# rll/rllab

Hardware: NVIDIA H100
Metric: env-steps/sec (full iteration: rollout + process_samples + VPG update) (higher is better)
Workload: dtype f32

## Files before the change

rllab_b200/csrc/tile_gram.cuh:

```cuda
#pragma once
#include "update_common.cuh"

namespace b200rl {

constexpr int TILE_AMAX = 6;
struct TileDist {
  float ls_new[TILE_AMAX], inv_std[TILE_AMAX], ls_old[TILE_AMAX], inv_std_old[TILE_AMAX], Mmu[TILE_AMAX],
      var_new[TILE_AMAX], var_new2[TILE_AMAX], var_old[TILE_AMAX];
  float sum_ls_new, sum_ls_old, half_log2pi_A;
};

template <class N, int MODE>
__device__ __forceinline__ void tile_dist_init(TileDist& D, const float* log_std_params, const UpdArgs& a) {
  constexpr int A = N::A;
  static_assert(A <= TILE_AMAX, "act_dim beyond the TileDist arrays");
  D.sum_ls_new = 0.f;
  D.sum_ls_old = 0.f;
#pragma unroll
  for (int k = 0; k < A; ++k) {
    D.ls_new[k] = clamp_log_std(log_std_params[k], a.log_min_std);
    const float sd = expf(D.ls_new[k]);
    D.inv_std[k] = 1.0f / sd;
    D.var_new[k] = sd * sd;
    D.var_new2[k] = 2.0f * sd * sd + 1e-8f;
    D.Mmu[k] = 2.0f / D.var_new2[k];
    D.ls_old[k] = (MODE == MODE_FVP) ? D.ls_new[k] : a.old_log_std[k];
    const float so = expf(D.ls_old[k]);
    D.inv_std_old[k] = 1.0f / so;
    D.var_old[k] = so * so;
    D.sum_ls_new += D.ls_new[k];
    D.sum_ls_old += D.ls_old[k];
  }
  D.half_log2pi_A = 0.5f * (float)A * 1.8378770664093453f;
}

template <class N, int RX, int RH1, int RH2, int RD1, int RD2, int RDM, int LD, bool PACKED = false, int TILE = 128>
struct TileGram {
  static constexpr int O = N::O, H = 32, A = N::A;
  static_assert(TILE == 128 || TILE == 64, "128- or 64-sample stages");
  static constexpr int WC = TILE == 128 ? 4 : 2;
  static constexpr int CS = 32 / WC;
  static constexpr int OQ = (O + 3) / 4;
  static_assert(N::H1 == 32 && N::H2 == 32 && A <= 6, "32-wide layers, act_dim <= 6");
  static constexpr int NS = A <= 3 ? 1 : 2;
  static constexpr int JDB = A <= 3 ? 3 : A;
  double accW1[4][WC];
  double accB[OQ + 1];
  double accA, accA1;
  double accT;
  float pA[NS][2], pT, pB[OQ + 1];

  __device__ __forceinline__ static void w1_tile_of(int tid, int& ti, int& tj, int& kh) {
    if constexpr (TILE == 128) {
      ti = (tid & 63) >> 3;
      tj = tid & 7;
      kh = tid >> 6;
    } else {
      ti = tid & 7;
      tj = tid >> 3;
      kh = 0;
    }
  }

  __device__ __forceinline__ void zero_partials() {
#pragma unroll
    for (int s = 0; s < NS; ++s) pA[s][0] = pA[s][1] = 0.f;
    pT = 0.f;
#pragma unroll
    for (int i = 0; i <= OQ; ++i) pB[i] = 0.f;
  }

  __device__ __forceinline__ void init() {
#pragma unroll
    for (int r = 0; r < 4; ++r)
#pragma unroll
      for (int c = 0; c < WC; ++c) accW1[r][c] = 0.0;
#pragma unroll
    for (int k = 0; k <= OQ; ++k) accB[k] = 0.0;
    accA = 0.0;
    accA1 = 0.0;
    accT = 0.0;
    zero_partials();
  }

  __device__ __forceinline__ void accumulate_a(const float* stage, int tid) {
    part_a(stage, tid);
    fold_a(tid);
  }
  __device__ __forceinline__ void accumulate_b(const float* stage, int tid) {
    part_b<LD>(stage, stage + RX * LD, tid);
    fold_b();
  }

  __device__ __forceinline__ void part_a(const float* stage, int tid) {
    int ti, tj, kh;
    w1_tile_of(tid, ti, tj, kh);
    const float* U = stage + (RH1 + ti) * LD + kh * 64;
    const float* V = stage + (RD2 + tj) * LD + kh * 64;
    if constexpr (PACKED) {
      float2 acc[4][WC];
#pragma unroll
      for (int r = 0; r < 4; ++r)
#pragma unroll
        for (int c = 0; c < WC; ++c) acc[r][c] = make_float2(0.f, 0.f);
#pragma unroll 2
      for (int k = 0; k < 64; k += 4) {
        float4 u[4], v[WC];
#pragma unroll
        for (int r = 0; r < 4; ++r) u[r] = *reinterpret_cast<const float4*>(U + r * 8 * LD + k);
#pragma unroll
        for (int c = 0; c < WC; ++c) v[c] = *reinterpret_cast<const float4*>(V + c * CS * LD + k);
#pragma unroll
        for (int r = 0; r < 4; ++r)
#pragma unroll
          for (int c = 0; c < WC; ++c) gram_fma4(u[r], v[c], acc[r][c]);
      }
#pragma unroll
      for (int r = 0; r < 4; ++r)
#pragma unroll
        for (int c = 0; c < WC; ++c) accW1[r][c] += (double)(acc[r][c].x + acc[r][c].y);
    } else {
      float acc[4][WC];
#pragma unroll
      for (int r = 0; r < 4; ++r)
#pragma unroll
        for (int c = 0; c < WC; ++c) acc[r][c] = 0.f;
#pragma unroll 4
      for (int k = 0; k < 64; k += 4) {
        float4 u[4], v[WC];
#pragma unroll
        for (int r = 0; r < 4; ++r) u[r] = *reinterpret_cast<const float4*>(U + r * 8 * LD + k);
#pragma unroll
        for (int c = 0; c < WC; ++c) v[c] = *reinterpret_cast<const float4*>(V + c * CS * LD + k);
#pragma unroll
        for (int r = 0; r < 4; ++r)
#pragma unroll
          for (int c = 0; c < WC; ++c) {
            acc[r][c] = fmaf(u[r].x, v[c].x, acc[r][c]);
            acc[r][c] = fmaf(u[r].y, v[c].y, acc[r][c]);
            acc[r][c] = fmaf(u[r].z, v[c].z, acc[r][c]);
            acc[r][c] = fmaf(u[r].w, v[c].w, acc[r][c]);
          }
      }
#pragma unroll
      for (int r = 0; r < 4; ++r)
#pragma unroll
        for (int c = 0; c < WC; ++c) accW1[r][c] += (double)acc[r][c];
    }
    const int lane = tid & 31, wq = tid >> 5;
#pragma unroll
    for (int s = 0; s < NS; ++s) {
    const int j = wq + 4 * s;
    if (j < A) {
      const float* Hh = stage + (RH2 + lane) * LD;
      const float* M = stage + (RDM + j) * LD;
      float s0 = pA[s][0], s1 = pA[s][1];
#pragma unroll 4
      for (int k = 0; k < TILE; k += 4) {
        const float4 hv = *reinterpret_cast<const float4*>(Hh + k);
        const float4 m = *reinterpret_cast<const float4*>(M + k);
        s0 = fmaf(hv.x, m.x, s0); s1 = fmaf(hv.y, m.y, s1);
        s0 = fmaf(hv.z, m.z, s0); s1 = fmaf(hv.w, m.w, s1);
      }
      pA[s][0] = s0;
      pA[s][1] = s1;
    } else if (j == JDB) {
      const float* Dr = stage + (RD2 + lane) * LD;
      float s0 = pA[s][0];
#pragma unroll 4
      for (int k = 0; k < TILE; k += 4) {
        const float4 d = *reinterpret_cast<const float4*>(Dr + k);
        s0 += (d.x + d.y) + (d.z + d.w);
      }
      pA[s][0] = s0;
    }
    }
    if (tid < 2 * A) {
      const float* Dr = stage + (RDM + tid) * LD;
      float s0 = pT;
#pragma unroll 4
      for (int k = 0; k < TILE; k += 4) {
        const float4 d = *reinterpret_cast<const float4*>(Dr + k);
        s0 += (d.x + d.y) + (d.z + d.w);
      }
      pT = s0;
    }
  }

  __device__ __forceinline__ void fold_a(int tid) {
    const int wq = tid >> 5;
#pragma unroll
    for (int s = 0; s < NS; ++s) {
      const int j = wq + 4 * s;
      double& acc = s == 0 ? accA : accA1;
      if (j < A) acc += (double)(pA[s][0] + pA[s][1]);
      else if (j == JDB) acc += (double)pA[s][0];
      pA[s][0] = pA[s][1] = 0.f;
    }
    if (tid < 2 * A) accT += (double)pT;
    pT = 0.f;
  }

  template <int XLD>
  __device__ __forceinline__ void part_b(const float* stage, const float* X, int tid) {
    const int lane = tid & 31, wq = tid >> 5;
    const float* Dr = stage + (RD1 + lane) * LD;
    float sa[OQ + 1];
#pragma unroll
    for (int i = 0; i <= OQ; ++i) sa[i] = pB[i];
#pragma unroll 4
    for (int k = 0; k < TILE; k += 4) {
      const float4 d = *reinterpret_cast<const float4*>(Dr + k);
#pragma unroll
      for (int i = 0; i < OQ; ++i) {
        const int o = wq + 4 * i;
        if (o < O) {
          const float4 xv = *reinterpret_cast<const float4*>(X + o * XLD + k);
          sa[i] = fmaf(xv.x, d.x, sa[i]); sa[i] = fmaf(xv.y, d.y, sa[i]);
          sa[i] = fmaf(xv.z, d.z, sa[i]); sa[i] = fmaf(xv.w, d.w, sa[i]);
        }
      }
      if (wq == 3) sa[OQ] += (d.x + d.y) + (d.z + d.w);
    }
#pragma unroll
    for (int i = 0; i <= OQ; ++i) pB[i] = sa[i];
  }

  __device__ __forceinline__ void fold_b() {
#pragma unroll
    for (int i = 0; i <= OQ; ++i) {
      accB[i] += (double)pB[i];
      pB[i] = 0.f;
    }
  }

  __device__ __forceinline__ void write(double* out, double* scr, int tid) {
    write(out, scr, tid, [] { __syncthreads(); });
  }
  template <class Sync>
  __device__ __forceinline__ void write(double* out, double* scr, int tid, Sync sync) {
    int ti, tj, kh;
    w1_tile_of(tid, ti, tj, kh);
    if constexpr (TILE == 128) {
      const int w1_tile = tid & 63;
#pragma unroll
      for (int r = 0; r < 4; ++r)
#pragma unroll
        for (int c = 0; c < 4; ++c) scr[(kh * 64 + w1_tile) * 16 + r * 4 + c] = accW1[r][c];
      sync();
      if (tid < 64) {
#pragma unroll
        for (int r = 0; r < 4; ++r)
#pragma unroll
          for (int c = 0; c < 4; ++c)
            out[N::oW1 + (ti + 8 * r) * H + (tj + 8 * c)] = scr[w1_tile * 16 + r * 4 + c] + scr[(64 + w1_tile) * 16 + r * 4 + c];
      }
    } else {
#pragma unroll
      for (int r = 0; r < 4; ++r)
#pragma unroll
        for (int c = 0; c < WC; ++c) out[N::oW1 + (ti + 8 * r) * H + (tj + CS * c)] = accW1[r][c];
    }
    const int lane = tid & 31, wq = tid >> 5;
#pragma unroll
    for (int i = 0; i < OQ; ++i) {
      const int o = wq + 4 * i;
      if (o < O) out[N::oW0 + o * H + lane] = accB[i];
    }
    if constexpr (A <= 3) {
      if (wq == 3) {
        out[N::ob0 + lane] = accB[OQ];
        out[N::ob1 + lane] = accA;
      } else if (wq < A) {
        out[N::oWo + lane * A + wq] = accA;
      }
    } else {
      if (wq == 3) out[N::ob0 + lane] = accB[OQ];
#pragma unroll
      for (int s = 0; s < NS; ++s) {
        const int j = wq + 4 * s;
        const double acc = s == 0 ? accA : accA1;
        if (j == JDB) out[N::ob1 + lane] = acc;
        else if (j < A) out[N::oWo + lane * A + j] = acc;
      }
    }
    if (tid < 2 * A) out[N::obo + tid] = accT;
  }
};

}
```

rllab_b200/csrc/update_umma32.cu:

```cuda
#include "tile_gram.cuh"
#include "umma_common.cuh"

namespace b200rl {

constexpr int V_THREADS = 128, V_TILE = 128, V_LD = V_TILE + 4;
#ifndef B200RL_V_PACKED_GRAM
#define B200RL_V_PACKED_GRAM 1
#endif
#ifndef B200RL_V_NWG_GRAD
#define B200RL_V_NWG_GRAD 4
#endif

template <class N, int MODE>
struct Umma32 {
  static constexpr int O = N::O, H = 32, A = N::A;
  static_assert(N::H1 == 32 && N::H2 == 32 && O <= 24, "tensor-core 32-wide kernel: (32,32) nets, obs_dim <= 24");
  static constexpr int KX = ((O + 7) / 8) * 8;
  static constexpr int IMG = 32 * 32 * 4, IMGX = 32 * KX * 4;
  static constexpr int o_bXT = 0, o_bW1T = o_bXT + 2 * IMGX, o_bW1 = o_bW1T + 2 * IMG,
                       o_bV1T = o_bW1 + (MODE == MODE_LOSS ? 0 : 2 * IMG),
                       o_img_end = o_bV1T + (MODE == MODE_FVP ? 2 * IMG : 0);
  static constexpr int n_small = ((64 + 2 * H * A + A + 3) / 4) * 4;
  static constexpr int o_small = o_img_end, o_stage = o_small + n_small * 4;
  static constexpr bool BLK = is_grad_mode(MODE) && A == 1;
  static constexpr int NB = BLK ? 1 : 2;
  static constexpr int NWG = BLK ? B200RL_V_NWG_GRAD : MODE == MODE_LOSS ? 3 : 2;
  static constexpr bool SEP_D1 = BLK && NWG <= 4;
  static constexpr int LD = NB * 64 + 4;
  static constexpr int rH1 = 0, rH2 = rH1 + H, rD2 = rH2 + H, rDM = rD2 + H, rDL = rDM + A,
                       rD1 = SEP_D1 ? rDL + A : rH2, R = (MODE == MODE_LOSS) ? 0 : SEP_D1 ? rD1 + H : rDL + A;
  static constexpr int RR = O + (MODE == MODE_FVP ? 0 : 2 * A + 1), qX = 0, qAct = O, qOm = O + A, qAdv = O + 2 * A;
  static constexpr int w_red = ((R * LD * 4 + 15) / 16) * 16, w_ring = w_red + 3 * 32 * 8,
                       w_bytes = w_ring + 2 * RR * V_LD * 4;
  static constexpr int o_dist = ((o_stage + 15) / 16) * 16;
  static constexpr int o_wg = ((o_dist + (int)sizeof(TileDist) + 15) / 16) * 16;
  static_assert(MODE == MODE_LOSS || BLK || 2 * 64 * 16 * 8 <= R * LD * 4, "stage region must hold the K-half combine scratch");
  static constexpr size_t bytes = (size_t)o_wg + (size_t)NWG * w_bytes;
  static_assert(bytes <= 232448, "does not fit the 227 KB of shared memory");
};

__device__ __forceinline__ void v_wg_sync(int wg) { asm volatile("bar.sync %0, 128;" ::"r"(wg + 1) : "memory"); }

template <int K, bool IS_MAX>
__device__ __forceinline__ void v_wg_reduce_store(const double (&v)[K], double* scratch, double* out, int tid, int wg) {
  const int lane = tid & 31, warp = tid >> 5;
#pragma unroll
  for (int k = 0; k < K; ++k) {
    double s = IS_MAX ? warp_max(v[k]) : warp_sum(v[k]);
    if (lane == 0) scratch[k * 32 + warp] = s;
  }
  v_wg_sync(wg);
  if (warp == 0) {
#pragma unroll
    for (int k = 0; k < K; ++k) {
      double s = lane < 4 ? scratch[k * 32 + lane] : (IS_MAX ? -1.0e300 : 0.0);
      s = IS_MAX ? warp_max(s) : warp_sum(s);
      if (lane == 0) out[k] = s;
    }
  }
  v_wg_sync(wg);
}

template <class SMT>
__device__ __forceinline__ void v_ring_load(const UpdArgs& a, float* ring, int slot, long long tile, int tid) {
  long long s = tile * V_TILE + tid;
  if (s >= a.B) s = a.B - 1;
  float* dst = ring + (size_t)slot * SMT::RR * V_LD + tid;
#pragma unroll
  for (int q = 0; q < SMT::RR; ++q) {
    const float* src = q < SMT::qAct ? a.obs + (size_t)q * a.B + s
                       : q < SMT::qOm ? a.act + (size_t)(q - SMT::qAct) * a.B + s
                       : q < SMT::qAdv ? a.old_mean + (size_t)(q - SMT::qOm) * a.B + s
                                       : a.adv + s;
    asm volatile("cp.async.ca.shared.global [%0], [%1], 4;" ::"r"(u_smem_u32(dst + q * V_LD)), "l"(src) : "memory");
  }
  asm volatile("cp.async.commit_group;" ::: "memory");
}

__device__ __forceinline__ int v_boff(int n, int k) {
  const int kp = u_kperm(k);
  return (kp & 3) * 4 + (n & 7) * 16 + (n >> 3) * 128 + (kp >> 2) * 512;
}

template <class N, int MODE>
__global__ void __launch_bounds__(V_THREADS * Umma32<N, MODE>::NWG, 1) update_umma32_kernel(UpdArgs a) {
  using SM = Umma32<N, MODE>;
  constexpr int O = N::O, H = 32, A = N::A, P = N::P, RLD = V_LD, LD = SM::LD, KX = SM::KX, KSX = KX / 8, NB = SM::NB;
  extern __shared__ __align__(1024) unsigned char smem[];
  float* small = reinterpret_cast<float*>(smem + SM::o_small);
  float* sb0 = small, *sb1 = small + H, *sWout = small + 2 * H, *sVout = sWout + H * A;
  float* sbo = (MODE == MODE_FVP) ? sVout + H * A : sWout + H * A;
  constexpr int NWG = SM::NWG, NT = NWG * V_THREADS;
  const int gtid = threadIdx.x, wg = gtid >> 7, tid = gtid & (V_THREADS - 1), warp = tid >> 5, lane = tid & 31, t4 = lane & 3;
  unsigned char* wreg = smem + SM::o_wg + (size_t)wg * SM::w_bytes;
  float* stage = reinterpret_cast<float*>(wreg);
  double* red_scratch = reinterpret_cast<double*>(wreg + SM::w_red);
  float* ring = reinterpret_cast<float*>(wreg + SM::w_ring);

  for (int e = gtid; e < H * H; e += NT) {
    const int i = e / H, j = e % H;
    const float w = a.params[N::oW1 + e];
    const float wh = tf32_hi(w);
    *reinterpret_cast<float*>(smem + SM::o_bW1T + v_boff(j, i)) = wh;
    *reinterpret_cast<float*>(smem + SM::o_bW1T + SM::IMG + v_boff(j, i)) = w - wh;
    if constexpr (MODE != MODE_LOSS) {
      *reinterpret_cast<float*>(smem + SM::o_bW1 + v_boff(i, j)) = wh;
      *reinterpret_cast<float*>(smem + SM::o_bW1 + SM::IMG + v_boff(i, j)) = w - wh;
    }
    if constexpr (MODE == MODE_FVP) {
      const float v = (float)a.xvec[N::oW1 + e];
      const float vh = tf32_hi(v);
      *reinterpret_cast<float*>(smem + SM::o_bV1T + v_boff(j, i)) = vh;
      *reinterpret_cast<float*>(smem + SM::o_bV1T + SM::IMG + v_boff(j, i)) = v - vh;
    }
  }
  for (int e = gtid; e < KX * H; e += NT) {
    const int o = e / H, j = e % H;
    float v = 0.f;
    if (o < O) v = (MODE == MODE_FVP) ? (float)a.xvec[N::oW0 + o * H + j] : a.params[N::oW0 + o * H + j];
    const float vh = tf32_hi(v);
    *reinterpret_cast<float*>(smem + SM::o_bXT + v_boff(j, o)) = vh;
    *reinterpret_cast<float*>(smem + SM::o_bXT + SM::IMGX + v_boff(j, o)) = v - vh;
  }
  for (int e = gtid; e < H * A; e += NT) {
    sWout[e] = a.params[N::oWo + e];
    if constexpr (MODE == MODE_FVP) sVout[e] = (float)a.xvec[N::oWo + e];
  }
  for (int e = gtid; e < H; e += NT) {
    sb0[e] = (MODE == MODE_FVP) ? (float)a.xvec[N::ob0 + e] : a.params[N::ob0 + e];
    sb1[e] = (MODE == MODE_FVP) ? (float)a.xvec[N::ob1 + e] : a.params[N::ob1 + e];
  }
  if (gtid < A) sbo[gtid] = (MODE == MODE_FVP) ? (float)a.xvec[N::obo + gtid] : a.params[N::obo + gtid];
  TileDist& D = *reinterpret_cast<TileDist*>(smem + SM::o_dist);
  if (gtid == 0) tile_dist_init<N, MODE>(D, a.params + N::ols, a);
  asm volatile("fence.proxy.async.shared::cta;" ::: "memory");
  __syncthreads();

  const uint32_t sbase = u_smem_u32(smem);
  auto gemm = [&](auto& acc, auto& f, int o_img, int img, int KS, bool accumulate) {
    constexpr int NV = sizeof(f[0]) / sizeof(float);
    const uint64_t b_hi = u_desc(sbase + o_img, 512, 128), b_lo = u_desc(sbase + o_img + img, 512, 128);
#pragma unroll
    for (int mb = 0; mb < NB; ++mb) {
      uint32_t hi[NV], lo[NV];
      u_to_operand(f[mb], hi, lo);
      wg_split_gemm(acc[mb], hi, lo, b_hi, b_lo, 1024, KS, accumulate);
    }
  };

  TileGram<N, 0, SM::rH1, SM::rH2, SM::rD1, SM::rD2, SM::rDM, LD, B200RL_V_PACKED_GRAM != 0, NB * 64> gram;
  if constexpr (MODE != MODE_LOSS) gram.init();
  double s_loss = 0.0, s_kl = 0.0, m_kl = -1.0e300;

  const int ntiles = (int)n_tiles_of(a, V_TILE), nvb = gridDim.x * NWG, vb = blockIdx.x * NWG + wg;
  if (vb < ntiles) v_ring_load<SM>(a, ring, 0, tile_at(a, vb), tid);
  int slot = 0;
  for (int ti_ = vb; ti_ < ntiles; ti_ += nvb, slot ^= 1) {
    const long long tile = tile_at(a, ti_);
    asm volatile("cp.async.wait_all;" ::: "memory");
    v_wg_sync(wg);
    if (ti_ + nvb < ntiles) v_ring_load<SM>(a, ring, slot ^ 1, tile_at(a, ti_ + nvb), tid);
#pragma unroll 1
    for (int b0 = 0; b0 < V_TILE; b0 += NB * 64) {
      const float* rs = ring + (size_t)slot * SM::RR * RLD + b0;
      int trow[NB][2];
      long long sl[NB][2];
      bool inrange[NB][2], valid[NB][2];
#pragma unroll
      for (int mb = 0; mb < NB; ++mb)
#pragma unroll
        for (int h = 0; h < 2; ++h) {
          trow[mb][h] = mb * 64 + warp * 16 + u_frag_row(2 * h, lane);
          const long long s = tile * V_TILE + b0 + trow[mb][h];
          inrange[mb][h] = s < a.B;
          valid[mb][h] = sample_valid(a, s);
          sl[mb][h] = inrange[mb][h] ? s : a.B - 1;
        }
      float accA[NB][16], accB[NB][16];
      {
        float xf[NB][4 * KSX];
#pragma unroll
        for (int mb = 0; mb < NB; ++mb)
#pragma unroll
          for (int i = 0; i < 4 * KSX; ++i) {
            const int o = u_frag_col(i, lane), h = (i >> 1) & 1;
            xf[mb][i] = o < O ? rs[(SM::qX + o) * RLD + trow[mb][h]] : 0.f;
          }
        if constexpr (MODE == MODE_FVP) {
          float h1f[NB][16];
#pragma unroll
          for (int mb = 0; mb < NB; ++mb)
#pragma unroll
            for (int i = 0; i < 16; ++i) {
              const int c = u_frag_col(i, lane), h = (i >> 1) & 1;
              h1f[mb][i] = a.h_cache[(size_t)c * a.B + sl[mb][h]];
              stage[(SM::rH1 + c) * LD + trow[mb][h]] = h1f[mb][i];
            }
          wg_fence();
          gemm(accA, xf, SM::o_bXT, SM::IMGX, KSX, false);
          gemm(accB, h1f, SM::o_bV1T, SM::IMG, 4, false);
          wg_commit();
        } else {
          wg_fence();
          gemm(accA, xf, SM::o_bXT, SM::IMGX, KSX, false);
          wg_commit();
        }
      }
      if (SM::SEP_D1 && b0 > 0) v_wg_sync(wg);
      wg_wait_all();
#pragma unroll
      for (int mb = 0; mb < NB; ++mb) {
        wg_fence_operand(accA[mb]);
        wg_fence_operand(accB[mb]);
      }
      {
        float v[NB][16];
#pragma unroll
        for (int mb = 0; mb < NB; ++mb)
#pragma unroll
          for (int i = 0; i < 16; ++i) {
            const int c = u_frag_col(i, lane), h = (i >> 1) & 1;
            if constexpr (MODE != MODE_FVP) {
              v[mb][i] = tanh_f(accA[mb][i] + sb0[c]);
              if constexpr (is_grad_mode(MODE)) {
                stage[(SM::rH1 + c) * LD + trow[mb][h]] = v[mb][i];
                if (a.h_cache != nullptr && inrange[mb][h]) a.h_cache[(size_t)c * a.B + sl[mb][h]] = v[mb][i];
              }
            } else {
              const float h1 = stage[(SM::rH1 + c) * LD + trow[mb][h]];
              v[mb][i] = (accA[mb][i] + sb0[c]) * (1.0f - h1 * h1);
            }
          }
        wg_fence();
        gemm(accB, v, SM::o_bW1T, SM::IMG, 4, MODE == MODE_FVP);
        wg_commit();
      }
      float h2f[NB][16];
      if constexpr (MODE == MODE_FVP) {
#pragma unroll
        for (int mb = 0; mb < NB; ++mb)
#pragma unroll
          for (int i = 0; i < 16; ++i)
            h2f[mb][i] = a.h_cache[(size_t)(H + u_frag_col(i, lane)) * a.B + sl[mb][(i >> 1) & 1]];
      }
      wg_wait_all();
#pragma unroll
      for (int mb = 0; mb < NB; ++mb) wg_fence_operand(accB[mb]);
      {
        float md[NB][2][A];
#pragma unroll
        for (int mb = 0; mb < NB; ++mb) {
#pragma unroll
          for (int h = 0; h < 2; ++h)
#pragma unroll
            for (int k = 0; k < A; ++k) md[mb][h][k] = 0.f;
#pragma unroll
          for (int i = 0; i < 16; ++i) {
            const int c = u_frag_col(i, lane), h = (i >> 1) & 1;
            if constexpr (MODE != MODE_FVP) {
              h2f[mb][i] = tanh_f(accB[mb][i] + sb1[c]);
              if constexpr (is_grad_mode(MODE)) {
                stage[(SM::rH2 + c) * LD + trow[mb][h]] = h2f[mb][i];
                if (a.h_cache != nullptr && inrange[mb][h]) a.h_cache[(size_t)(H + c) * a.B + sl[mb][h]] = h2f[mb][i];
              }
#pragma unroll
              for (int k = 0; k < A; ++k) md[mb][h][k] = fmaf(h2f[mb][i], sWout[c * A + k], md[mb][h][k]);
            } else {
              stage[(SM::rH2 + c) * LD + trow[mb][h]] = h2f[mb][i];
              const float t2 = (accB[mb][i] + sb1[c]) * (1.0f - h2f[mb][i] * h2f[mb][i]);
#pragma unroll
              for (int k = 0; k < A; ++k)
                md[mb][h][k] = fmaf(t2, sWout[c * A + k], fmaf(h2f[mb][i], sVout[c * A + k], md[mb][h][k]));
            }
          }
        }
#pragma unroll
        for (int mb = 0; mb < NB; ++mb)
#pragma unroll
          for (int h = 0; h < 2; ++h)
#pragma unroll
            for (int k = 0; k < A; ++k) {
              md[mb][h][k] += __shfl_xor_sync(0xffffffffu, md[mb][h][k], 1);
              md[mb][h][k] += __shfl_xor_sync(0xffffffffu, md[mb][h][k], 2);
            }
        float dmu[NB][2][A];
#pragma unroll
        for (int mb = 0; mb < NB; ++mb)
#pragma unroll
          for (int h = 0; h < 2; ++h) {
            const int r = trow[mb][h];
            if constexpr (MODE != MODE_FVP) {
              float act[A], om[A];
#pragma unroll
              for (int k = 0; k < A; ++k) {
                act[k] = rs[(SM::qAct + k) * RLD + r];
                om[k] = rs[(SM::qOm + k) * RLD + r];
              }
              const float adv_s = rs[SM::qAdv * RLD + r];
              float z[A], zz[A], dmk[A], zsq = 0.f, zsq_old = 0.f, kl = 0.f;
#pragma unroll
              for (int k = 0; k < A; ++k) {
                const float mu = sbo[k] + md[mb][h][k];
                z[k] = (act[k] - mu) * D.inv_std[k];
                zz[k] = __fmul_rn(z[k], z[k]);
                zsq += zz[k];
                const float zo = (act[k] - om[k]) * D.inv_std_old[k];
                zsq_old += zo * zo;
                const float dm = om[k] - mu;
                dmk[k] = dm;
                kl += (dm * dm + D.var_old[k] - D.var_new[k]) / D.var_new2[k] + D.ls_new[k] - D.ls_old[k];
              }
              const float logp_new = -D.sum_ls_new - 0.5f * zsq - D.half_log2pi_A;
              float w_s, term;
              if (a.loss_kind == B200RL_LOSS_TRPO) {
                const float logp_old = -D.sum_ls_old - 0.5f * zsq_old - D.half_log2pi_A;
                w_s = expf(logp_new - logp_old) * adv_s;
                term = -w_s;
              } else {
                w_s = adv_s;
                term = -logp_new * adv_s;
              }
              if (!valid[mb][h]) { w_s = 0.f; term = 0.f; }
              if (t4 == 0) {
                s_loss += (double)term;
                if (valid[mb][h]) { s_kl += (double)kl; m_kl = fmax(m_kl, (double)kl); }
              }
              if constexpr (is_grad_mode(MODE)) {
#pragma unroll
                for (int k = 0; k < A; ++k) {
                  dmu[mb][h][k] = -w_s * z[k] * D.inv_std[k];
                  if constexpr (MODE == MODE_GRAD_KL) {
                    float dls = -w_s * (zz[k] - 1.0f);
                    if (valid[mb][h])
                      add_kl_penalty(a.penalty, dmk[k], D.var_new[k], D.var_new2[k], D.var_old[k], dmu[mb][h][k], dls);
                    if (t4 == 0) {
                      stage[(SM::rDM + k) * LD + r] = dmu[mb][h][k];
                      stage[(SM::rDL + k) * LD + r] = dls;
                    }
                  } else if (t4 == 0) {
                    stage[(SM::rDM + k) * LD + r] = dmu[mb][h][k];
                    stage[(SM::rDL + k) * LD + r] = -w_s * (zz[k] - 1.0f);
                  }
                }
              }
            } else {
#pragma unroll
              for (int k = 0; k < A; ++k) {
                dmu[mb][h][k] = valid[mb][h] ? (sbo[k] + md[mb][h][k]) * D.Mmu[k] : 0.f;
                if (t4 == 0) {
                  stage[(SM::rDM + k) * LD + r] = dmu[mb][h][k];
                  stage[(SM::rDL + k) * LD + r] = 0.f;
                }
              }
            }
          }
        if constexpr (MODE != MODE_LOSS) {
          float v[NB][16];
#pragma unroll
          for (int mb = 0; mb < NB; ++mb)
#pragma unroll
            for (int i = 0; i < 16; ++i) {
              const int c = u_frag_col(i, lane), h = (i >> 1) & 1;
              float sacc = 0.f;
#pragma unroll
              for (int k = 0; k < A; ++k) sacc = fmaf(dmu[mb][h][k], sWout[c * A + k], sacc);
              v[mb][i] = sacc * (1.0f - h2f[mb][i] * h2f[mb][i]);
              stage[(SM::rD2 + c) * LD + trow[mb][h]] = v[mb][i];
            }
          wg_fence();
          gemm(accA, v, SM::o_bW1, SM::IMG, 4, false);
          wg_commit();
        }
      }
      if constexpr (MODE != MODE_LOSS) {
        auto e3 = [&] {
#pragma unroll
          for (int mb = 0; mb < NB; ++mb)
#pragma unroll
            for (int i = 0; i < 16; ++i) {
              const int c = u_frag_col(i, lane), r = trow[mb][(i >> 1) & 1];
              const float h1 = stage[(SM::rH1 + c) * LD + r];
              stage[(SM::rD1 + c) * LD + r] = accA[mb][i] * (1.0f - h1 * h1);
            }
        };
        if constexpr (SM::SEP_D1) {
          wg_wait_all();
#pragma unroll
          for (int mb = 0; mb < NB; ++mb) wg_fence_operand(accA[mb]);
          e3();
          v_wg_sync(wg);
          gram.part_a(stage, tid);
          gram.template part_b<RLD>(stage, rs + SM::qX * RLD, tid);
        } else {
          constexpr bool wait_first = NWG >= 3;
          if constexpr (wait_first) {
            wg_wait_all();
#pragma unroll
            for (int mb = 0; mb < NB; ++mb) wg_fence_operand(accA[mb]);
          }
          v_wg_sync(wg);
          gram.part_a(stage, tid);
          v_wg_sync(wg);
          if constexpr (!wait_first) {
            wg_wait_all();
#pragma unroll
            for (int mb = 0; mb < NB; ++mb) wg_fence_operand(accA[mb]);
          }
          e3();
          v_wg_sync(wg);
          gram.template part_b<RLD>(stage, rs + SM::qX * RLD, tid);
          v_wg_sync(wg);
        }
      }
    }
    if constexpr (MODE != MODE_LOSS) {
      gram.fold_a(tid);
      gram.fold_b();
    }
  }

  if constexpr (MODE != MODE_LOSS) {
    double* out = a.partial + (size_t)vb * P;
    gram.write(out, reinterpret_cast<double*>(stage), tid, [wg] { v_wg_sync(wg); });
  }
  if constexpr (MODE != MODE_FVP) {
    double v[2] = {s_loss, s_kl};
    double mx[1] = {m_kl};
    double* sc = a.partial + (is_grad_mode(MODE) ? (size_t)nvb * P : (size_t)0) + (size_t)vb * 3;
    v_wg_reduce_store<2, false>(v, red_scratch, sc, tid, wg);
    v_wg_reduce_store<1, true>(mx, red_scratch, sc + 2, tid, wg);
  }
}

template <class N, int MODE>
static int launch_umma32(const UpdArgs& a, int* grid_out, cudaStream_t st) {
  using SM = Umma32<N, MODE>;
  B200RL_SET_MAX_SMEM((update_umma32_kernel<N, MODE>), SM::bytes);
  long long grid = num_sms();
  const long long ntiles = host_n_tiles(a, V_TILE);
  if (grid > (ntiles + SM::NWG - 1) / SM::NWG) grid = (ntiles + SM::NWG - 1) / SM::NWG;
  if (grid > MAX_PARTIAL_BLOCKS / SM::NWG) grid = MAX_PARTIAL_BLOCKS / SM::NWG;
  if (grid < 1) grid = 1;
  update_umma32_kernel<N, MODE><<<(unsigned)grid, V_THREADS * SM::NWG, SM::bytes, st>>>(a);
  B200RL_LAUNCH_CHECK("update_umma32_kernel");
  *grid_out = (int)grid * SM::NWG;
  return 0;
}

int update_umma32_launch(int mode, int obs_dim, int act_dim, const UpdArgs& a, int* grid_out, int* P_out, int* ols_out,
                         cudaStream_t st) {
  const int h1 = 32, h2 = 32;
  B200RL_DISPATCH_NET_H(32, {
    *P_out = NetT::P;
    *ols_out = NetT::ols;
    int rc = (mode == MODE_GRAD)      ? launch_umma32<NetT, MODE_GRAD>(a, grid_out, st)
             : (mode == MODE_GRAD_KL) ? launch_umma32<NetT, MODE_GRAD_KL>(a, grid_out, st)
             : (mode == MODE_LOSS)    ? launch_umma32<NetT, MODE_LOSS>(a, grid_out, st)
                                      : launch_umma32<NetT, MODE_FVP>(a, grid_out, st);
    if (rc) return rc;
  });
  return 0;
}

}
```

Measured before the change: 2.192 billion.

## Move W1 gram accumulators to shared memory to fit five warpgroups

Adds a W1S mode in TileGram that keeps the double-precision W1, bias-0 and output-bias accumulators in per-warpgroup shared memory instead of registers, used when the grad kernel runs without separate D1 staging. Raises the default grad warpgroup count from 4 to 5 (only for small observation dims) to increase concurrent tiles per SM. It also folds the loss, KL-sum and KL-max scalars into a single register spread across lanes t4 = 0, 1 and 2, combined with shuffles at the end. The trade-off is extra shared-memory traffic and a larger footprint per warpgroup in exchange for lower register pressure and more parallelism.

```diff
diff --git a/rllab_b200/csrc/tile_gram.cuh b/rllab_b200/csrc/tile_gram.cuh
--- a/rllab_b200/csrc/tile_gram.cuh
+++ b/rllab_b200/csrc/tile_gram.cuh
@@ -34,16 +34,19 @@
   D.half_log2pi_A = 0.5f * (float)A * 1.8378770664093453f;
 }
 
-template <class N, int RX, int RH1, int RH2, int RD1, int RD2, int RDM, int LD, bool PACKED = false, int TILE = 128>
+template <class N, int RX, int RH1, int RH2, int RD1, int RD2, int RDM, int LD, bool PACKED = false, int TILE = 128,
+          bool W1S = false>
 struct TileGram {
   static constexpr int O = N::O, H = 32, A = N::A;
   static_assert(TILE == 128 || TILE == 64, "128- or 64-sample stages");
+  static_assert(!W1S || TILE == 64, "shared-memory accumulators for 64-sample stages");
   static constexpr int WC = TILE == 128 ? 4 : 2;
   static constexpr int CS = 32 / WC;
   static constexpr int OQ = (O + 3) / 4;
   static_assert(N::H1 == 32 && N::H2 == 32 && A <= 6, "32-wide layers, act_dim <= 6");
   static constexpr int NS = A <= 3 ? 1 : 2;
   static constexpr int JDB = A <= 3 ? 3 : A;
+  static constexpr int W1S_T = 32 * 32, W1S_B0 = W1S_T + 3 * A, W1S_DOUBLES = W1S_B0 + 32;
   double accW1[4][WC];
   double accB[OQ + 1];
   double accA, accA1;
@@ -62,6 +65,23 @@
     }
   }
 
+  __device__ __forceinline__ double& w1_acc(double* w1s, int tid, int r, int c) {
+    if constexpr (W1S) return w1s[(r * WC + c) * 128 + tid];
+    else return accW1[r][c];
+  }
+  __device__ __forceinline__ double& t_acc(double* w1s, int tid) {
+    if constexpr (W1S) return w1s[W1S_T + tid];
+    else return accT;
+  }
+  __device__ __forceinline__ float& t_part(double* w1s, int tid) {
+    if constexpr (W1S) return reinterpret_cast<float*>(w1s + W1S_T + 2 * A)[tid];
+    else return pT;
+  }
+  __device__ __forceinline__ double& b0_acc(double* w1s, int tid) {
+    if constexpr (W1S) return w1s[W1S_B0 + (tid & 31)];
+    else return accB[OQ];
+  }
+
   __device__ __forceinline__ void zero_partials() {
 #pragma unroll
     for (int s = 0; s < NS; ++s) pA[s][0] = pA[s][1] = 0.f;
@@ -70,13 +90,18 @@
     for (int i = 0; i <= OQ; ++i) pB[i] = 0.f;
   }
 
-  __device__ __forceinline__ void init() {
+  __device__ __forceinline__ void init(double* w1s = nullptr, int tid = 0) {
 #pragma unroll
     for (int r = 0; r < 4; ++r)
 #pragma unroll
-      for (int c = 0; c < WC; ++c) accW1[r][c] = 0.0;
-#pragma unroll
-    for (int k = 0; k <= OQ; ++k) accB[k] = 0.0;
+      for (int c = 0; c < WC; ++c) w1_acc(w1s, tid, r, c) = 0.0;
+    if (W1S && tid < 2 * A) {
+      t_acc(w1s, tid) = 0.0;
+      t_part(w1s, tid) = 0.f;
+    }
+#pragma unroll
+    for (int k = 0; k < OQ; ++k) accB[k] = 0.0;
+    if (!W1S || (tid >> 5) == 3) b0_acc(w1s, tid) = 0.0;
     accA = 0.0;
     accA1 = 0.0;
     accT = 0.0;
@@ -92,7 +117,7 @@
     fold_b();
   }
 
-  __device__ __forceinline__ void part_a(const float* stage, int tid) {
+  __device__ __forceinline__ void part_a(const float* stage, int tid, double* w1s = nullptr) {
     int ti, tj, kh;
     w1_tile_of(tid, ti, tj, kh);
     const float* U = stage + (RH1 + ti) * LD + kh * 64;
@@ -103,7 +128,7 @@
       for (int r = 0; r < 4; ++r)
 #pragma unroll
         for (int c = 0; c < WC; ++c) acc[r][c] = make_float2(0.f, 0.f);
-#pragma unroll 2
+#pragma unroll (W1S ? 1 : 2)
       for (int k = 0; k < 64; k += 4) {
         float4 u[4], v[WC];
 #pragma unroll
@@ -118,7 +143,7 @@
 #pragma unroll
       for (int r = 0; r < 4; ++r)
 #pragma unroll
-        for (int c = 0; c < WC; ++c) accW1[r][c] += (double)(acc[r][c].x + acc[r][c].y);
+        for (int c = 0; c < WC; ++c) w1_acc(w1s, tid, r, c) += (double)(acc[r][c].x + acc[r][c].y);
     } else {
       float acc[4][WC];
 #pragma unroll
@@ -145,7 +170,7 @@
 #pragma unroll
       for (int r = 0; r < 4; ++r)
 #pragma unroll
-        for (int c = 0; c < WC; ++c) accW1[r][c] += (double)acc[r][c];
+        for (int c = 0; c < WC; ++c) w1_acc(w1s, tid, r, c) += (double)acc[r][c];
     }
     const int lane = tid & 31, wq = tid >> 5;
 #pragma unroll
@@ -177,17 +202,17 @@
     }
     if (tid < 2 * A) {
       const float* Dr = stage + (RDM + tid) * LD;
-      float s0 = pT;
+      float s0 = t_part(w1s, tid);
 #pragma unroll 4
       for (int k = 0; k < TILE; k += 4) {
         const float4 d = *reinterpret_cast<const float4*>(Dr + k);
         s0 += (d.x + d.y) + (d.z + d.w);
       }
-      pT = s0;
-    }
-  }
-
-  __device__ __forceinline__ void fold_a(int tid) {
+      t_part(w1s, tid) = s0;
+    }
+  }
+
+  __device__ __forceinline__ void fold_a(int tid, double* w1s = nullptr) {
     const int wq = tid >> 5;
 #pragma unroll
     for (int s = 0; s < NS; ++s) {
@@ -197,8 +222,10 @@
       else if (j == JDB) acc += (double)pA[s][0];
       pA[s][0] = pA[s][1] = 0.f;
     }
-    if (tid < 2 * A) accT += (double)pT;
-    pT = 0.f;
+    if (tid < 2 * A) {
+      t_acc(w1s, tid) += (double)t_part(w1s, tid);
+      t_part(w1s, tid) = 0.f;
+    }
   }
 
   template <int XLD>
@@ -226,19 +253,21 @@
     for (int i = 0; i <= OQ; ++i) pB[i] = sa[i];
   }
 
-  __device__ __forceinline__ void fold_b() {
-#pragma unroll
-    for (int i = 0; i <= OQ; ++i) {
+  __device__ __forceinline__ void fold_b(int tid = 0, double* w1s = nullptr) {
+#pragma unroll
+    for (int i = 0; i < OQ; ++i) {
       accB[i] += (double)pB[i];
       pB[i] = 0.f;
     }
+    if (!W1S || (tid >> 5) == 3) b0_acc(w1s, tid) += (double)pB[OQ];
+    pB[OQ] = 0.f;
   }
 
   __device__ __forceinline__ void write(double* out, double* scr, int tid) {
     write(out, scr, tid, [] { __syncthreads(); });
   }
   template <class Sync>
-  __device__ __forceinline__ void write(double* out, double* scr, int tid, Sync sync) {
+  __device__ __forceinline__ void write(double* out, double* scr, int tid, Sync sync, double* w1s = nullptr) {
     int ti, tj, kh;
     w1_tile_of(tid, ti, tj, kh);
     if constexpr (TILE == 128) {
@@ -259,7 +288,7 @@
 #pragma unroll
       for (int r = 0; r < 4; ++r)
 #pragma unroll
-        for (int c = 0; c < WC; ++c) out[N::oW1 + (ti + 8 * r) * H + (tj + CS * c)] = accW1[r][c];
+        for (int c = 0; c < WC; ++c) out[N::oW1 + (ti + 8 * r) * H + (tj + CS * c)] = w1_acc(w1s, tid, r, c);
     }
     const int lane = tid & 31, wq = tid >> 5;
 #pragma unroll
@@ -269,13 +298,13 @@
     }
     if constexpr (A <= 3) {
       if (wq == 3) {
-        out[N::ob0 + lane] = accB[OQ];
+        out[N::ob0 + lane] = b0_acc(w1s, tid);
         out[N::ob1 + lane] = accA;
       } else if (wq < A) {
         out[N::oWo + lane * A + wq] = accA;
       }
     } else {
-      if (wq == 3) out[N::ob0 + lane] = accB[OQ];
+      if (wq == 3) out[N::ob0 + lane] = b0_acc(w1s, tid);
 #pragma unroll
       for (int s = 0; s < NS; ++s) {
         const int j = wq + 4 * s;
@@ -284,7 +313,7 @@
         else if (j < A) out[N::oWo + lane * A + j] = acc;
       }
     }
-    if (tid < 2 * A) out[N::obo + tid] = accT;
+    if (tid < 2 * A) out[N::obo + tid] = t_acc(w1s, tid);
   }
 };
 
diff --git a/rllab_b200/csrc/update_umma32.cu b/rllab_b200/csrc/update_umma32.cu
--- a/rllab_b200/csrc/update_umma32.cu
+++ b/rllab_b200/csrc/update_umma32.cu
@@ -8,7 +8,7 @@
 #define B200RL_V_PACKED_GRAM 1
 #endif
 #ifndef B200RL_V_NWG_GRAD
-#define B200RL_V_NWG_GRAD 4
+#define B200RL_V_NWG_GRAD 5
 #endif
 
 template <class N, int MODE>
@@ -24,13 +24,16 @@
   static constexpr int o_small = o_img_end, o_stage = o_small + n_small * 4;
   static constexpr bool BLK = is_grad_mode(MODE) && A == 1;
   static constexpr int NB = BLK ? 1 : 2;
-  static constexpr int NWG = BLK ? B200RL_V_NWG_GRAD : MODE == MODE_LOSS ? 3 : 2;
-  static constexpr bool SEP_D1 = BLK && NWG <= 4;
+  static constexpr int NWG = BLK ? (B200RL_V_NWG_GRAD > 4 && O > 4 ? 4 : B200RL_V_NWG_GRAD) : MODE == MODE_LOSS ? 3 : 2;
+  static constexpr bool SEP_D1 = BLK && NWG <= 4, W1S = BLK && !SEP_D1;
   static constexpr int LD = NB * 64 + 4;
   static constexpr int rH1 = 0, rH2 = rH1 + H, rD2 = rH2 + H, rDM = rD2 + H, rDL = rDM + A,
                        rD1 = SEP_D1 ? rDL + A : rH2, R = (MODE == MODE_LOSS) ? 0 : SEP_D1 ? rD1 + H : rDL + A;
   static constexpr int RR = O + (MODE == MODE_FVP ? 0 : 2 * A + 1), qX = 0, qAct = O, qOm = O + A, qAdv = O + 2 * A;
-  static constexpr int w_red = ((R * LD * 4 + 15) / 16) * 16, w_ring = w_red + 3 * 32 * 8,
+  using Gram = TileGram<N, 0, rH1, rH2, rD1, rD2, rDM, LD, B200RL_V_PACKED_GRAM != 0, NB * 64, W1S>;
+  static constexpr int w_stage = ((R * LD * 4 + 15) / 16) * 16, w_red = W1S ? 0 : w_stage,
+                       w_w1 = W1S ? w_stage : w_stage + 3 * 32 * 8,
+                       w_ring = w_w1 + (W1S ? ((Gram::W1S_DOUBLES * 8 + 15) / 16) * 16 : 0),
                        w_bytes = w_ring + 2 * RR * V_LD * 4;
   static constexpr int o_dist = ((o_stage + 15) / 16) * 16;
   static constexpr int o_wg = ((o_dist + (int)sizeof(TileDist) + 15) / 16) * 16;
@@ -95,6 +98,7 @@
   unsigned char* wreg = smem + SM::o_wg + (size_t)wg * SM::w_bytes;
   float* stage = reinterpret_cast<float*>(wreg);
   double* red_scratch = reinterpret_cast<double*>(wreg + SM::w_red);
+  double* w1s = SM::W1S ? reinterpret_cast<double*>(wreg + SM::w_w1) : nullptr;
   float* ring = reinterpret_cast<float*>(wreg + SM::w_ring);
 
   for (int e = gtid; e < H * H; e += NT) {
@@ -148,9 +152,9 @@
     }
   };
 
-  TileGram<N, 0, SM::rH1, SM::rH2, SM::rD1, SM::rD2, SM::rDM, LD, B200RL_V_PACKED_GRAM != 0, NB * 64> gram;
-  if constexpr (MODE != MODE_LOSS) gram.init();
-  double s_loss = 0.0, s_kl = 0.0, m_kl = -1.0e300;
+  typename SM::Gram gram;
+  if constexpr (MODE != MODE_LOSS) gram.init(w1s, tid);
+  double lacc = t4 == 2 ? -1.0e300 : 0.0;
 
   const int ntiles = (int)n_tiles_of(a, V_TILE), nvb = gridDim.x * NWG, vb = blockIdx.x * NWG + wg;
   if (vb < ntiles) v_ring_load<SM>(a, ring, 0, tile_at(a, vb), tid);
@@ -321,9 +325,12 @@
                 term = -logp_new * adv_s;
               }
               if (!valid[mb][h]) { w_s = 0.f; term = 0.f; }
-              if (t4 == 0) {
-                s_loss += (double)term;
-                if (valid[mb][h]) { s_kl += (double)kl; m_kl = fmax(m_kl, (double)kl); }
+              if constexpr (SM::W1S) {
+                if (t4 < 2) lacc += (double)(t4 == 0 ? term : valid[mb][h] ? kl : 0.f);
+                else if (valid[mb][h]) lacc = fmax(lacc, (double)kl);
+              } else {
+                const double lx = (double)(t4 == 0 ? term : valid[mb][h] ? kl : 0.f);
+                lacc = t4 != 2 ? lacc + lx : valid[mb][h] ? fmax(lacc, lx) : lacc;
               }
               if constexpr (is_grad_mode(MODE)) {
 #pragma unroll
@@ -399,7 +406,7 @@
             for (int mb = 0; mb < NB; ++mb) wg_fence_operand(accA[mb]);
           }
           v_wg_sync(wg);
-          gram.part_a(stage, tid);
+          gram.part_a(stage, tid, w1s);
           v_wg_sync(wg);
           if constexpr (!wait_first) {
             wg_wait_all();
@@ -414,18 +421,19 @@
       }
     }
     if constexpr (MODE != MODE_LOSS) {
-      gram.fold_a(tid);
-      gram.fold_b();
+      gram.fold_a(tid, w1s);
+      gram.fold_b(tid, w1s);
     }
   }
 
   if constexpr (MODE != MODE_LOSS) {
     double* out = a.partial + (size_t)vb * P;
-    gram.write(out, reinterpret_cast<double*>(stage), tid, [wg] { v_wg_sync(wg); });
+    gram.write(out, reinterpret_cast<double*>(stage), tid, [wg] { v_wg_sync(wg); }, w1s);
   }
   if constexpr (MODE != MODE_FVP) {
-    double v[2] = {s_loss, s_kl};
-    double mx[1] = {m_kl};
+    const double kl_sum = __shfl_down_sync(0xffffffffu, lacc, 1), kl_max = __shfl_down_sync(0xffffffffu, lacc, 2);
+    double v[2] = {t4 == 0 ? lacc : 0.0, t4 == 0 ? kl_sum : 0.0};
+    double mx[1] = {t4 == 0 ? kl_max : -1.0e300};
     double* sc = a.partial + (is_grad_mode(MODE) ? (size_t)nvb * P : (size_t)0) + (size_t)vb * 3;
     v_wg_reduce_store<2, false>(v, red_scratch, sc, tid, wg);
     v_wg_reduce_store<1, true>(mx, red_scratch, sc + 2, tid, wg);
```

New measurement: 2.234 billion (median of 6 runs). 1.9% higher.
